# Alvin-Zeng/DRN

Measured on AMD Instinct MI355X. Metric: clips/sec fwd+bwd (BxT=256x4096 C3D feats), higher is better.
Workload: dtype bf16; 1 GPU; Charades-STA-shaped C3D features, T=256, D=4096, batch 32/GPU, stage-1 losses; step = fwd+bwd+grad all-reduce+clip(0.5)+Adam; global_batch=32, T=256, D=4096, parallelism=dp1

## Files before the change

drn_amd/csrc/api.hip:

```cpp
#include <stdarg.h>
#include "common.h"
#include "../../include/drn_hip.h"

static thread_local char g_err[512] = "";

void drn_set_error(const char* fmt, ...) {
  va_list ap;
  va_start(ap, fmt);
  vsnprintf(g_err, sizeof(g_err), fmt, ap);
  va_end(ap);
}

extern "C" int drn_abi_version(void) {
  drn_clear_status(); return DRN_ABI_VERSION; }
extern "C" const char* drn_last_error(void) { return g_err; }

static int g_tune[16] = {4096, 1, 256, 0, 0, 0, 0, 0, 1, 1, 0, 16, 160, 512, 2048, 1};
int drn_tuning(int key) { return g_tune[key]; }
extern "C" int drn_tune(const char* key, int value) {
  drn_clear_status();
  if (key && !strcmp(key, "tn3_minrows")) { g_tune[DRN_TUNE_TN3_MINROWS] = value; return DRN_OK; }
  if (key && !strcmp(key, "tn_fused")) { g_tune[DRN_TUNE_TN_FUSED] = value; return DRN_OK; }
  if (key && !strcmp(key, "nt_w4c")) { g_tune[DRN_TUNE_NT_W4C] = value; return DRN_OK; }
  if (key && !strcmp(key, "nt_w4")) { g_tune[DRN_TUNE_NT_W4] = value; return DRN_OK; }
  if (key && !strcmp(key, "nt_deep")) { g_tune[DRN_TUNE_NT_DEEP] = value; return DRN_OK; }
  if (key && !strcmp(key, "nt_w4h")) { g_tune[DRN_TUNE_NT_W4H] = value; return DRN_OK; }
  if (key && !strcmp(key, "w4h_tapil")) { g_tune[DRN_TUNE_W4H_TAPIL] = value; return DRN_OK; }
  if (key && !strcmp(key, "w4h_halo")) { g_tune[DRN_TUNE_W4H_HALO] = value; return DRN_OK; }
  if (key && !strcmp(key, "bn1_maxwg")) { g_tune[DRN_TUNE_BN1_MAXWG] = value; return DRN_OK; }
  if (key && !strcmp(key, "nt_deep2")) { g_tune[DRN_TUNE_NT_DEEP2] = value; return DRN_OK; }
  if (key && !strcmp(key, "nt_deep_ks")) { g_tune[DRN_TUNE_NT_DEEP_KS] = value; return DRN_OK; }
  if (key && !strncmp(key, "exp", 3) && key[3] >= '0' && key[3] <= '4' && !key[4]) { g_tune[DRN_TUNE_EXP0 + (key[3] - '0')] = value; return DRN_OK; }
  drn_set_error("drn_tune: unknown key %s", key ? key : "(null)");
  return DRN_ERR_ARG;
}
```

drn_amd/csrc/common.h:

```cpp
#pragma once
#include <hip/hip_runtime.h>
#include <stdint.h>
#include <stdio.h>
#include <string.h>

#define DRN_OK 0
#define DRN_ERR_ARG (-1)
#define DRN_ERR_LAUNCH (-2)
#define DRN_ERR_UNSUPPORTED (-3)

#define DRN_F32 0
#define DRN_BF16 1

typedef __bf16 bf16_t;
typedef __bf16 bf16x8 __attribute__((ext_vector_type(8)));
typedef __bf16 bf16x4 __attribute__((ext_vector_type(4)));
typedef short s16x4 __attribute__((ext_vector_type(4)));
typedef float f32x4 __attribute__((ext_vector_type(4)));
typedef float f32x2 __attribute__((ext_vector_type(2)));

template <typename T>
__device__ __forceinline__ T* as_global(T* p) {
  typedef __attribute__((address_space(1))) T* g_t;
  g_t g = (g_t)p;
  asm("" : "+s"(g));
  return (T*)g;
}
template <typename T>
__device__ __forceinline__ T* as_global_v(T* p) {
  typedef __attribute__((address_space(1))) T* g_t;
  g_t g = (g_t)p;
  asm("" : "+v"(g));
  return (T*)g;
}


void drn_set_error(const char* fmt, ...);

#define DRN_CHECK_ARG(cond, ...)          \
  do {                                    \
    if (!(cond)) {                        \
      drn_set_error(__VA_ARGS__);         \
      return DRN_ERR_ARG;                 \
    }                                     \
  } while (0)

static inline void drn_clear_status() { (void)hipGetLastError(); }

static inline int drn_launch_status(const char* what) {
  hipError_t e = hipGetLastError();
  if (e != hipSuccess) {
    drn_set_error("%s: launch failed: %s", what, hipGetErrorString(e));
    return DRN_ERR_LAUNCH;
  }
  return DRN_OK;
}

static inline int cdiv(int a, int b) { return (a + b - 1) / b; }

#ifdef DRN_EXPERIMENTS
#include <stdlib.h>
static inline const char* drn_exp_env(const char* name) { return getenv(name); }
#else
static inline const char* drn_exp_env(const char*) { return nullptr; }
#endif
int drn_tuning(int key);
#define DRN_XCHG_CONFIRM 0x20000
#define DRN_XCHG_READBACK 0x40000
#define DRN_XCHG_NONE 0x80000
#define DRN_TUNE_TN3_MINROWS 0
#define DRN_TUNE_TN_FUSED 1
#define DRN_TUNE_EXP0 3
#define DRN_TUNE_NT_W4C 9
#define DRN_TUNE_NT_W4 8
#define DRN_TUNE_NT_DEEP 2
#define DRN_TUNE_NT_W4H 12
#define DRN_TUNE_BN1_MAXWG 13
#define DRN_TUNE_W4H_TAPIL 14
#define DRN_TUNE_W4H_HALO 15
#define DRN_TUNE_NT_DEEP2 10
#define DRN_TUNE_NT_DEEP_KS 11

static __device__ uint4 g_zero_page[4];

template <typename T> struct DT;
template <> struct DT<float> {
  static __device__ __forceinline__ float ld(const float* p) { return *p; }
  static __device__ __forceinline__ void st(float* p, float v) { *p = v; }
  static __device__ __forceinline__ float round(float v) { return v; }
};
template <> struct DT<bf16_t> {
  static __device__ __forceinline__ float ld(const bf16_t* p) { return (float)*p; }
  static __device__ __forceinline__ void st(bf16_t* p, float v) { *p = (bf16_t)v; }
  static __device__ __forceinline__ float round(float v) { return (float)(bf16_t)v; }
};

__device__ __forceinline__ float wave_sum(float v) {
#pragma unroll
  for (int o = 32; o > 0; o >>= 1) v += __shfl_xor(v, o, 64);
  return v;
}

__device__ __forceinline__ float block_sum(float v, float* sh ) {
  v = wave_sum(v);
  const int w = threadIdx.x >> 6, l = threadIdx.x & 63, nw = blockDim.x >> 6;
  __syncthreads();
  if (l == 0) sh[w] = v;
  __syncthreads();
  if (w == 0) {
    float t = l < nw ? sh[l] : 0.f;
    t = wave_sum(t);
    if (l == 0) sh[16] = t;
  }
  __syncthreads();
  return sh[16];
}
```

drn_amd/csrc/gemm_tn.hip:

```cpp
#include <stdlib.h>
#include <type_traits>
#include "common.h"
#include "../../include/drn_hip.h"



struct WgradGroup {
  const void* dY;
  const void* X;
  int M, Lout, Lsrc, ldy, ldx;
  int blk_start;
};
struct WgradParams {
  int ngroups;
  WgradGroup g[DRN_MAX_GROUPS];
  int total_blks, blks_per_split;
  int N, Cin, taps, stride, pad;
  int ctiles;
  float* out;
  int direct;
  int w_layout;
  int accumulate;
  int multi;
  int z_start[DRN_MAX_GROUPS + 1], bps[DRN_MAX_GROUPS], gdirect[DRN_MAX_GROUPS];
// ... 238 lines not shown
        if (c >= Cin) continue;
        float v = acc[mi][ni][r];
        if (direct) {
          float* dst = P.w_layout == 0 ? out_ptr + ((long)n * KW + tap * Cin + c)
                                       : out_ptr + ((long)n * KW + (long)c * P.taps + tap);
          if (P.accumulate) v += *dst;
          *dst = v;
        } else {
          out_ptr[((long)split * P.N + n) * KW + tap * Cin + c] = v;
        }
      }
    }
}

__device__ __forceinline__ bf16x8 tr_frag(const char* lo_addr, const char* hi_addr) {
  typedef __attribute__((address_space(3))) s16x4* lp;
  union { struct { s16x4 a, b; } s; bf16x8 v; } u;
  u.s.a = __builtin_amdgcn_ds_read_tr16_b64_v4i16((lp)lo_addr);
  u.s.b = __builtin_amdgcn_ds_read_tr16_b64_v4i16((lp)hi_addr);
  return u.v;
}

template <int NSTG>
__global__ __launch_bounds__(512, 2) void conv_wgrad3_tn_kernel(const WgradParams P) {
  extern __shared__ __attribute__((aligned(16))) char smem[];
  typedef bf16_t T;
  constexpr int R = 64, MI = 4, NI = 2;
  constexpr int IMG = 16384, HALO_B = 512, STAGE_B = 2 * IMG + HALO_B;
  const int tid = threadIdx.x, w = __builtin_amdgcn_readfirstlane(tid >> 6), l = tid & 63;
  const int n0 = blockIdx.x * 128, c0 = blockIdx.y * 128;
  int split = blockIdx.z;
  int blk_lo = split * P.blks_per_split;
  int blk_hi = min(blk_lo + P.blks_per_split, P.total_blks);
  float* out_ptr = P.out;
  int direct = P.direct;
  if (P.multi) {
    int pg = 0;
#pragma unroll
    for (int i = 1; i < DRN_MAX_GROUPS; ++i)
      if (i < P.ngroups && (int)blockIdx.z >= P.z_start[i]) pg = i;
    split = blockIdx.z - P.z_start[pg];
    const int blk_end = pg + 1 < P.ngroups ? P.g[pg + 1].blk_start : P.total_blks;
    blk_lo = P.g[pg].blk_start + split * P.bps[pg];
    blk_hi = min(blk_lo + P.bps[pg], blk_end);
    out_ptr = P.gout[pg];
    direct = P.gdirect[pg];
  }
  const T* zero = (const T*)g_zero_page;

  const int srow = w * 8 + (l >> 3);
  const int scol = (((l & 7) >> 1) ^ ((srow >> 1) & 3)) * 16 + (l & 1) * 8;
  long y_off[2], x_off[2];
#pragma unroll
  for (int j = 0; j < 2; ++j) {
    y_off[j] = n0 + j * 64 + scol < P.N ? n0 + j * 64 + scol : -1;
    x_off[j] = c0 + j * 64 + scol < P.Cin ? c0 + j * 64 + scol : -1;
  }
  const bool is_halo = (w == 0) & (l < 32);
  const int hcol = ((l >> 3) & 1) * 64 + (l & 7) * 8;
  const long xh_off = c0 + hcol < P.Cin ? c0 + hcol : -1;
  const int rowoff[2] = {srow, (l >> 4) ? R : -1};
  int s_blk = blk_lo, s_g = 0;
#pragma unroll
  for (int i = 1; i < DRN_MAX_GROUPS; ++i)
    if (i < P.ngroups && blk_lo >= P.g[i].blk_start) s_g = i;
  int s_seq[2], s_t[2];
  const T* g_Y;
  const T* g_X;
  int g_L, g_nseq, g_ldy, g_ldx, g_next;
  auto locate = [&]() {
    const WgradGroup& G = P.g[s_g];
    g_Y = (const T*)G.dY;
    g_X = (const T*)G.X;
    g_L = G.Lout;
    g_nseq = G.M / G.Lout;
    g_ldy = G.ldy;
    g_ldx = G.ldx;
    g_next = s_g + 1 < P.ngroups ? P.g[s_g + 1].blk_start : 0x7fffffff;
    const int Lp = G.Lout + 1;
    const int pbase = (s_blk - G.blk_start) * R;
#pragma unroll
    for (int j = 0; j < 2; ++j) {
      const int p = pbase + rowoff[j] + Lp;
      const int q = p / Lp;
      s_seq[j] = q - 1;
      s_t[j] = p - q * Lp;
    }
  };
  locate();

  auto row_ptr = [&](const T* base, int m, int ld, long coff, bool ok) -> const T* {
    const unsigned off = __umul24((unsigned)m, (unsigned)ld) + (unsigned)coff;
    const T* p = base + off;
    return ok ? p : zero;
  };
  auto stage_part = [&](int buf, int part) {
    char* Ys = smem + buf * STAGE_B;
    char* Xs = Ys + IMG;
    char* Hs = Xs + IMG;
    const bool live = s_blk < blk_hi;
    const int L = g_L;
    const bool ok = live & ((unsigned)s_seq[0] < (unsigned)g_nseq) & (s_t[0] < L);
    const int m = s_seq[0] * L + s_t[0];
    if (part == 0) glds16(row_ptr(g_Y, m, g_ldy, y_off[0], ok & (y_off[0] >= 0)), Ys + w * 1024);
    if (part == 1) glds16(row_ptr(g_X, m, g_ldx, x_off[0], ok & (x_off[0] >= 0)), Xs + w * 1024);
    if (part == 2) glds16(row_ptr(g_Y, m, g_ldy, y_off[1], ok & (y_off[1] >= 0)), Ys + 8192 + w * 1024);
    if (part == 3) {
      glds16(row_ptr(g_X, m, g_ldx, x_off[1], ok & (x_off[1] >= 0)), Xs + 8192 + w * 1024);
      if (is_halo) {
        const bool okh = live & ((unsigned)s_seq[1] < (unsigned)g_nseq) & (s_t[1] < L) & (xh_off >= 0);
        glds16(row_ptr(g_X, s_seq[1] * L + s_t[1], g_ldx, xh_off, okh), Hs);
      }
    }
    if (part != 4) return;
    ++s_blk;
    if (s_blk >= g_next) {
      ++s_g;
      locate();
    } else {
      const int Lp = L + 1;
      if (Lp > R) {
#pragma unroll
        for (int j = 0; j < 2; ++j) {
          s_t[j] += R;
          const bool wrap = s_t[j] >= Lp;
          s_t[j] -= wrap ? Lp : 0;
          s_seq[j] += wrap ? 1 : 0;
        }
      } else {
#pragma unroll
        for (int j = 0; j < 2; ++j) {
          s_t[j] += R;
          while (s_t[j] >= Lp) {
            s_t[j] -= Lp;
            ++s_seq[j];
          }
        }
      }
    }
  };
  auto stage = [&](int buf) {
#pragma unroll
    for (int part = 0; part < 5; ++part) stage_part(buf, part);
  };

  f32x4 acc[3][MI][NI];
#pragma unroll
  for (int t = 0; t < 3; ++t)
#pragma unroll
    for (int mi = 0; mi < MI; ++mi)
#pragma unroll
      for (int ni = 0; ni < NI; ++ni) acc[t][mi][ni] = (f32x4){0.f, 0.f, 0.f, 0.f};
  const int wr = w >> 2, wc = w & 3;

  const int fr = (l >> 4) * 4 + ((l & 15) >> 2);
  const int fb = (l & 3) * 8;
  int ya[MI], xa[3][NI], x_first[NI], x_last[NI];
#pragma unroll
  for (int mi = 0; mi < MI; ++mi) ya[mi] = wr * 8192 + fr * 128 + ((mi ^ ((fr >> 1) & 3)) * 32) + fb;
#pragma unroll
  for (int ni = 0; ni < NI; ++ni) {
    const int half = wc >> 1, cb = (wc & 1) * 2 + ni;
#pragma unroll
    for (int t = 0; t < 3; ++t) {
      const int rr = fr + t - 1;
      xa[t][ni] = IMG + half * 8192 + rr * 128 + ((cb ^ ((rr >> 1) & 3)) * 32) + fb;
    }
    x_first[ni] = fr == 0 ? 2 * IMG + half * 128 + cb * 32 + fb : xa[0][ni];
    x_last[ni] = fr == 15 ? 2 * IMG + 256 + half * 128 + cb * 32 + fb : xa[2][ni] + 4096 + 2048;
  }

  struct Frags {
    bf16x8 a[MI], b[3][NI];
  };
  auto load_frags = [&](Frags& F, const char* S, auto ks_) {
    constexpr int ks = decltype(ks_)::value;
#pragma unroll
    for (int mi = 0; mi < MI; ++mi) {
      const char* q = S + ya[mi] + ks * 4096;
      F.a[mi] = tr_frag(q, q + 2048);
    }
#pragma unroll
    for (int ni = 0; ni < NI; ++ni) {
      const char* q0 = S + xa[0][ni] + ks * 4096;
      const char* q1 = S + xa[1][ni] + ks * 4096;
      const char* q2 = S + xa[2][ni] + ks * 4096;
      F.b[1][ni] = tr_frag(q1, q1 + 2048);
      F.b[0][ni] = tr_frag(ks == 0 ? S + x_first[ni] : q0, q0 + 2048);
      F.b[2][ni] = tr_frag(q2, ks == 1 ? S + x_last[ni] : q2 + 2048);
    }
  };
  auto mfma_frags = [&](const Frags& F, int mi0) {
#pragma unroll
    for (int t = 0; t < 3; ++t)
#pragma unroll
      for (int mi = 0; mi < 2; ++mi)
#pragma unroll
        for (int ni = 0; ni < NI; ++ni)
          acc[t][mi0 + mi][ni] = __builtin_amdgcn_mfma_f32_16x16x32_bf16(F.a[mi0 + mi], F.b[t][ni], acc[t][mi0 + mi][ni], 0, 0, 0);
  };
  typedef std::integral_constant<int, 0> K0;
  typedef std::integral_constant<int, 1> K1;

  auto wait_landed = [&](int younger) {
    if (younger <= 0) asm volatile("s_waitcnt vmcnt(0)" ::: "memory");
    else if (younger == 1) { if (w == 0) asm volatile("s_waitcnt vmcnt(5)" ::: "memory"); else asm volatile("s_waitcnt vmcnt(4)" ::: "memory"); }
    else { if (w == 0) asm volatile("s_waitcnt vmcnt(10)" ::: "memory"); else asm volatile("s_waitcnt vmcnt(8)" ::: "memory"); }
  };
#pragma unroll
  for (int st = 0; st < NSTG - 1; ++st) stage(st);
  wait_landed(NSTG - 2);
  __builtin_amdgcn_s_barrier();
  asm volatile("" ::: "memory");
  Frags F0, F1;
  load_frags(F0, smem, K0());
  int cur = 0;
  for (int blk = blk_lo; blk < blk_hi; ++blk) {
    wait_landed(NSTG - 3);
    __builtin_amdgcn_s_barrier();
    asm volatile("" ::: "memory");
    int nxt = cur + NSTG - 1;
    if (nxt >= NSTG) nxt -= NSTG;
    const int cn = cur + 1 == NSTG ? 0 : cur + 1;
    load_frags(F1, smem + cur * STAGE_B, K1());
    stage_part(nxt, 0);
    __builtin_amdgcn_sched_barrier(0);
    mfma_frags(F0, 0);
    __builtin_amdgcn_sched_barrier(0);
    stage_part(nxt, 1);
    __builtin_amdgcn_sched_barrier(0);
    mfma_frags(F0, 2);
    __builtin_amdgcn_sched_barrier(0);
    load_frags(F0, smem + cn * STAGE_B, K0());
    stage_part(nxt, 2);
    __builtin_amdgcn_sched_barrier(0);
    mfma_frags(F1, 0);
    __builtin_amdgcn_sched_barrier(0);
    stage_part(nxt, 3);
    __builtin_amdgcn_sched_barrier(0);
    mfma_frags(F1, 2);
    __builtin_amdgcn_sched_barrier(0);
    stage_part(nxt, 4);
    cur = cn;
  }
  asm volatile("s_waitcnt vmcnt(0)" ::: "memory");

  const int KW = 3 * P.Cin;
  const bool rowmajor = !direct || (P.w_layout == 0 && !P.accumulate);
  float* obase = direct ? out_ptr : out_ptr + (long)split * P.N * KW;
  if (rowmajor && (P.Cin % 4 == 0) && (((uintptr_t)obase & 15) == 0)) {
    constexpr int PITCH = 32 * 4 + 16;
    __syncthreads();
    char* wbuf = smem + w * (32 * PITCH);
#pragma unroll
    for (int t = 0; t < 3; ++t)
#pragma unroll
      for (int ch = 0; ch < MI / 2; ++ch) {
        const int nrow0 = n0 + wr * 64 + ch * 32;
#pragma unroll
        for (int mi2 = 0; mi2 < 2; ++mi2)
#pragma unroll
          for (int r = 0; r < 4; ++r)
#pragma unroll
            for (int ni = 0; ni < NI; ++ni)
              *((float*)(wbuf + (mi2 * 16 + (l >> 4) * 4 + r) * PITCH) + ni * 16 + (l & 15)) = acc[t][ch * 2 + mi2][ni][r];
        asm volatile("s_waitcnt lgkmcnt(0)" ::: "memory");
#pragma unroll
        for (int it = 0; it < 4; ++it) {
          const int rl = it * 8 + (l >> 3), cv = l & 7;
          const int n = nrow0 + rl, c = c0 + wc * 32 + cv * 4;
          if (n < P.N && c < P.Cin) {
            const f32x4 v = *(const f32x4*)(wbuf + rl * PITCH + cv * 16);
            *(f32x4*)(obase + ((long)n * KW + t * P.Cin + c)) = v;
          }
        }
        asm volatile("s_waitcnt lgkmcnt(0)" ::: "memory");
      }
    return;
  }
#pragma unroll
  for (int t = 0; t < 3; ++t)
#pragma unroll
    for (int mi = 0; mi < MI; ++mi)
#pragma unroll
      for (int r = 0; r < 4; ++r) {
        const int n = n0 + wr * 64 + mi * 16 + (l >> 4) * 4 + r;
        if (n >= P.N) continue;
#pragma unroll
        for (int ni = 0; ni < NI; ++ni) {
          const int c = c0 + wc * 32 + ni * 16 + (l & 15);
          if (c >= P.Cin) continue;
          float v = acc[t][mi][ni][r];
          if (direct) {
            float* dst = P.w_layout == 0 ? out_ptr + ((long)n * KW + t * P.Cin + c) : out_ptr + ((long)n * KW + (long)c * 3 + t);
            if (P.accumulate) v += *dst;
            *dst = v;
          } else {
            out_ptr[((long)split * P.N + n) * KW + t * P.Cin + c] = v;
          }
        }
      }
}

struct WgradReduceMulti {
  const float* ws[DRN_MAX_GROUPS];
  float* out[DRN_MAX_GROUPS];
  int nsplit[DRN_MAX_GROUPS];
  int cin[DRN_MAX_GROUPS];
};
__global__ void wgrad_reduce_multi_kernel(const WgradReduceMulti R, int N, int taps, int w_layout, int accumulate) {
  const int Cin = R.cin[blockIdx.y];
  const long KW = (long)taps * Cin;
  const long total = (long)N * KW;
  const float* __restrict__ ws = R.ws[blockIdx.y];
  float* __restrict__ out = R.out[blockIdx.y];
  const int nsplit = R.nsplit[blockIdx.y];
  if (nsplit <= 1) return;
  if (w_layout == 1 && taps == 3) {
    const long pairs = (long)N * Cin;
    for (long idx = (long)blockIdx.x * blockDim.x + threadIdx.x; idx < pairs; idx += (long)gridDim.x * blockDim.x) {
      const long n = idx / Cin;
      const int c = (int)(idx - n * Cin);
      const float* p = ws + n * KW + c;
      float s0 = 0.f, s1 = 0.f, s2 = 0.f;
#pragma unroll 4
      for (int z = 0; z < nsplit; ++z) {
        s0 += p[(long)z * total];
        s1 += p[(long)z * total + Cin];
        s2 += p[(long)z * total + 2 * Cin];
      }
      float* o = out + n * KW + (long)c * 3;
      if (accumulate) {
        s0 += o[0];
        s1 += o[1];
        s2 += o[2];
      }
      o[0] = s0;
      o[1] = s1;
      o[2] = s2;
    }
    return;
  }
  for (long idx = (long)blockIdx.x * blockDim.x + threadIdx.x; idx < total; idx += (long)gridDim.x * blockDim.x) {
    float s = 0.f;
    for (int z = 0; z < nsplit; ++z) s += ws[(long)z * total + idx];
    long o = idx;
    if (w_layout == 1) {
      const long n = idx / KW;
      const int rem = (int)(idx - n * KW);
      const int tap = rem / Cin, c = rem - tap * Cin;
      o = n * KW + (long)c * taps + tap;
    }
    if (accumulate) s += out[o];
    out[o] = s;
  }
}

__global__ void wgrad_reduce_kernel(const float* __restrict__ ws, float* __restrict__ out, int nsplit, int N, int Cin,
                                    int taps, int w_layout, int accumulate) {
  const long KW = (long)taps * Cin;
  const long total = (long)N * KW;
  if (w_layout == 1 && taps == 3) {
    const long pairs = (long)N * Cin;
    for (long idx = (long)blockIdx.x * blockDim.x + threadIdx.x; idx < pairs; idx += (long)gridDim.x * blockDim.x) {
      const long n = idx / Cin;
      const int c = (int)(idx - n * Cin);
      const float* p = ws + n * KW + c;
      float s0 = 0.f, s1 = 0.f, s2 = 0.f;
#pragma unroll 4
      for (int z = 0; z < nsplit; ++z) {
        s0 += p[(long)z * total];
        s1 += p[(long)z * total + Cin];
        s2 += p[(long)z * total + 2 * Cin];
      }
      float* o = out + n * KW + (long)c * 3;
      if (accumulate) {
        s0 += o[0];
        s1 += o[1];
        s2 += o[2];
      }
      o[0] = s0;
      o[1] = s1;
      o[2] = s2;
    }
    return;
  }
  for (long idx = (long)blockIdx.x * blockDim.x + threadIdx.x; idx < total; idx += (long)gridDim.x * blockDim.x) {
    float s = 0.f;
    for (int z = 0; z < nsplit; ++z) s += ws[(long)z * total + idx];
    long o = idx;
    if (w_layout == 1) {
      const long n = idx / KW;
      const int rem = (int)(idx - n * KW);
      const int tap = rem / Cin, c = rem - tap * Cin;
      o = n * KW + (long)c * taps + tap;
    }
    if (accumulate) s += out[o];
    out[o] = s;
  }
}

typedef DrnWgradPendItem WgradPendItem;
#define WGRAD_PEND_MAX DRN_WGRAD_PEND_MAX
typedef DrnWgradPending WgradPendParams;

static int wgrad_pend_push(DrnWgradPending* L, const float* ws, float* out, int nsplit, int N, int Cin, int taps, int w_layout, int accumulate) {
  if (!L || L->n < 0 || L->n >= WGRAD_PEND_MAX) return 0;
  for (int i = 0; i < L->n; ++i)
    if (L->it[i].out == out) {
      drn_set_error("drn_gemm_wgrad: the output already has a deferred reduce pending in this DrnWgradPending (flush with drn_wgrad_reduce_pending first)");
      return DRN_ERR_ARG;
    }
  if (accumulate) return 0;
  L->it[L->n++] = WgradPendItem{ws, out, nsplit, N, Cin, taps, w_layout, accumulate};
  return 1;
}

__global__ __launch_bounds__(256) void wgrad_reduce_all_kernel(const WgradPendParams P) {
  __shared__ float sh_sq[17];
  float sq = 0.f;
  int i = 0;
  for (int k = 1; k < P.n; ++k)
    if ((int)blockIdx.x >= P.blk_start[k]) i = k;
  const WgradPendItem& I = P.it[i];
  const int nb = P.blk_start[i + 1] - P.blk_start[i], b = blockIdx.x - P.blk_start[i];
  const float* __restrict__ ws = I.ws;
  float* __restrict__ out = I.out;
  const int N = I.N, Cin = I.Cin, taps = I.taps, nsplit = I.nsplit, accumulate = I.accumulate, w_layout = I.w_layout;
  const long KW = (long)taps * Cin;
  const long total = (long)N * KW;
  if (w_layout == 1 && taps == 3) {
    const long pairs = (long)N * Cin;
    for (long idx = (long)b * 256 + threadIdx.x; idx < pairs; idx += (long)nb * 256) {
      const long n = idx / Cin;
      const int c = (int)(idx - n * Cin);
      const float* p = ws + n * KW + c;
      float s0 = 0.f, s1 = 0.f, s2 = 0.f;
#pragma unroll 4
      for (int z = 0; z < nsplit; ++z) {
        s0 += __builtin_nontemporal_load(p + (long)z * total);
        s1 += __builtin_nontemporal_load(p + (long)z * total + Cin);
        s2 += __builtin_nontemporal_load(p + (long)z * total + 2 * Cin);
      }
      float* o = out + n * KW + (long)c * 3;
      if (accumulate) {
        s0 += o[0];
        s1 += o[1];
        s2 += o[2];
      }
      o[0] = s0;
      o[1] = s1;
      o[2] = s2;
      sq = fmaf(s0, s0, sq); sq = fmaf(s1, s1, sq); sq = fmaf(s2, s2, sq);
    }
  } else {
    for (long idx = (long)b * 256 + threadIdx.x; idx < total; idx += (long)nb * 256) {
      float s = 0.f;
      for (int z = 0; z < nsplit; ++z) s += __builtin_nontemporal_load(ws + (long)z * total + idx);
      long o = idx;
      if (w_layout == 1) {
        const long n = idx / KW;
        const int rem = (int)(idx - n * KW);
        const int tap = rem / Cin, c = rem - tap * Cin;
        o = n * KW + (long)c * taps + tap;
      }
      if (accumulate) s += out[o];
      out[o] = s;
      sq = fmaf(s, s, sq);
    }
  }
  if (P.sumsq) {
    sq = block_sum(sq, sh_sq);
    if (threadIdx.x == 0) P.sumsq[blockIdx.x] = sq;
  }
}

static int wgrad_pend_plan(DrnWgradPending* L) {
  int blocks = 0;
  for (int i = 0; i < L->n; ++i) {
    const WgradPendItem& I = L->it[i];
    const long work = (I.w_layout == 1 && I.taps == 3) ? (long)I.N * I.Cin : (long)I.N * I.taps * I.Cin;
    int nb = (int)((work + 255) / 256);
    if (nb > 2048) nb = 2048;
    L->blk_start[i] = blocks;
    blocks += nb;
  }
  L->blk_start[L->n] = blocks;
  return blocks;
}

extern "C" int drn_wgrad_pending_blocks(DrnWgradPending* L) {
  drn_clear_status();
  DRN_CHECK_ARG(L && L->n >= 0 && L->n <= WGRAD_PEND_MAX, "drn_wgrad_pending_blocks: bad list");
  return wgrad_pend_plan(L);
}

extern "C" int64_t drn_wgrad_pending_bytes(const DrnWgradPending* L) {
  int64_t b = 0;
  if (!L || L->n < 0 || L->n > WGRAD_PEND_MAX) return 0;
  for (int i = 0; i < L->n; ++i) {
    const WgradPendItem& I = L->it[i];
    b += (int64_t)I.N * I.taps * I.Cin * 4 * (I.nsplit + 1 + (I.accumulate ? 1 : 0));
  }
  return b;
}

extern "C" int drn_wgrad_reduce_pending(DrnWgradPending* L, float* sumsq, void* stream) {
  drn_clear_status();
  DRN_CHECK_ARG(L && L->n >= 0 && L->n <= WGRAD_PEND_MAX, "drn_wgrad_reduce_pending: bad list");
  if (L->n == 0) return DRN_OK;
  const int blocks = wgrad_pend_plan(L);
  L->sumsq = sumsq;
  wgrad_reduce_all_kernel<<<blocks, 256, 0, (hipStream_t)stream>>>(*L);
  L->n = 0;
  L->sumsq = nullptr;
  return drn_launch_status("drn_wgrad_reduce_pending");
}

static int wgrad_tile(int N, int Cin, int taps) {
  if (const char* e = drn_exp_env("DRN_TN_TILE")) return atoi(e) == 256 ? 256 : 128;
  return (long)cdiv(N, 256) * taps * cdiv(Cin, 256) >= 128 ? 256 : 128;
}

static int wgrad_nsplit(int total_blks, int N, int Cin, int taps) {
  const int tile = wgrad_tile(N, Cin, taps);
  const int tiles = cdiv(N, tile) * taps * cdiv(Cin, tile);
  const int tgt = drn_tuning(DRN_TUNE_EXP0 + 2) > 0 ? drn_tuning(DRN_TUNE_EXP0 + 2) : 768;
  int ns = cdiv(tile == 256 ? 256 : tgt, tiles);
  const int cap = total_blks / 12;
  if (ns > cap) ns = cap;
  if (ns < 1) ns = 1;
  if (ns > 64) ns = 64;
  return ns;
}

static int total_blocks_upper(int M_total, int ngroups_max) {
  return cdiv(M_total, 32) + ngroups_max;
}

static int wgrad3_nsplit(int m_total, int N, int Cin) {
  int target = drn_tuning(DRN_TUNE_EXP0 + 1) > 0 ? drn_tuning(DRN_TUNE_EXP0 + 1) : 256;
  if (const char* e = drn_exp_env("DRN_TN3_TARGET")) target = atoi(e);
  const int tiles = cdiv(N, 128) * cdiv(Cin, 128);
  int ns = target / tiles;
  const int cap = cdiv(m_total, 64) / 8;
  if (ns > cap) ns = cap;
  if (ns < 1) ns = 1;
  if (ns > 64) ns = 64;
  return ns;
}
static bool wgrad3_enabled() {
  return drn_tuning(DRN_TUNE_TN_FUSED) != 0;
}
static bool wgrad3_group_ok(const DrnWgradDesc& s) {
  return s.Lsrc == s.Lout && s.M < (1 << 24) && s.ldy < (1 << 24) && s.ldx < (1 << 24) &&
         (long)s.M * s.ldy < (1L << 31) && (long)s.M * s.ldx < (1L << 31);
}
static int wgrad3_min_rows() {
  return drn_tuning(DRN_TUNE_TN3_MINROWS);
}
static void wgrad3_attr() {
  static bool set = false;
  if (!set) {
#ifdef DRN_EXPERIMENTS
    (void)hipFuncSetAttribute((const void*)conv_wgrad3_tn_kernel<3>, hipFuncAttributeMaxDynamicSharedMemorySize, 163840);
#endif
    (void)hipFuncSetAttribute((const void*)conv_wgrad3_tn_kernel<4>, hipFuncAttributeMaxDynamicSharedMemorySize, 163840);
    set = true;
  }
}
#define WGRAD3_STAGE (2 * 16384 + 512)
static int wgrad3_stages() {
  int st = 4;
  if (const char* e = drn_exp_env("DRN_TN3_STAGES")) st = atoi(e);
  return st < 3 ? 3 : (st > 4 ? 4 : st);
}
#ifdef DRN_EXPERIMENTS
#define WGRAD3_LAUNCH(GRID, P) do { const int st_ = wgrad3_stages(); \
    if (st_ == 3) conv_wgrad3_tn_kernel<3><<<GRID, 512, 3 * WGRAD3_STAGE, stream>>>(P); \
    else conv_wgrad3_tn_kernel<4><<<GRID, 512, 4 * WGRAD3_STAGE, stream>>>(P); } while (0)
#else
#define WGRAD3_LAUNCH(GRID, P) conv_wgrad3_tn_kernel<4><<<GRID, 512, 4 * WGRAD3_STAGE, stream>>>(P)
#endif

extern "C" int64_t drn_wgrad_ws_elems(int M_total, int N, int Cin, int taps) {
  int ns = wgrad_nsplit(total_blocks_upper(M_total, DRN_MAX_GROUPS), N, Cin, taps);
  if (taps == 3) {
    const int ns3 = wgrad3_nsplit(M_total, N, Cin);
    if (ns3 > ns) ns = ns3;
  }
  return ns > 1 ? (int64_t)ns * N * taps * Cin : 0;
}

extern "C" int drn_gemm_wgrad(const DrnWgradDesc* d, int ngroups, float* dW, int N, int Cin, int taps, int stride, int pad,
                              int w_layout, int accumulate, float* ws, int dtype, DrnWgradPending* pend, void* stream_) {
  drn_clear_status();
  hipStream_t stream = (hipStream_t)stream_;
  DRN_CHECK_ARG(ngroups >= 1 && ngroups <= DRN_MAX_GROUPS, "drn_gemm_wgrad: ngroups=%d out of range", ngroups);
  DRN_CHECK_ARG(dtype == DRN_F32 || dtype == DRN_BF16, "drn_gemm_wgrad: bad dtype %d", dtype);
  DRN_CHECK_ARG(dW && N > 0 && Cin > 0 && taps >= 1 && stride >= 1, "drn_gemm_wgrad: bad dims");
  if (pend)
    for (int i = 0; i < pend->n && i < WGRAD_PEND_MAX; ++i)
      DRN_CHECK_ARG(pend->it[i].out != dW, "drn_gemm_wgrad: the output already has a deferred reduce pending in this DrnWgradPending (flush first)");
  const int ch = dtype == DRN_BF16 ? 8 : 4;
  const int R = dtype == DRN_BF16 ? 64 : 32;
  WgradParams P;
  memset(&P, 0, sizeof(P));
  P.ngroups = ngroups;
  int blks = 0, m_total = 0;
  for (int g = 0; g < ngroups; ++g) {
    const DrnWgradDesc& s = d[g];
    DRN_CHECK_ARG(s.dY && s.X && s.M > 0 && s.Lout > 0 && s.Lsrc > 0 && s.M % s.Lout == 0, "drn_gemm_wgrad: bad group %d", g);
    DRN_CHECK_ARG(s.ldy % ch == 0 && s.ldx % ch == 0 && N % ch == 0 && Cin % ch == 0,
                  "drn_gemm_wgrad: N/Cin/ldy/ldx must be multiples of %d elements", ch);
    DRN_CHECK_ARG(((uintptr_t)s.dY & 15) == 0 && ((uintptr_t)s.X & 15) == 0, "drn_gemm_wgrad: operands must be 16-byte aligned");
    P.g[g].dY = s.dY; P.g[g].X = s.X; P.g[g].M = s.M; P.g[g].Lout = s.Lout; P.g[g].Lsrc = s.Lsrc;
    P.g[g].ldy = s.ldy; P.g[g].ldx = s.ldx; P.g[g].blk_start = blks;
    blks += cdiv(s.M, R);
    m_total += s.M;
  }
  bool fused = dtype == DRN_BF16 && taps == 3 && stride == 1 && pad == 1 && wgrad3_enabled() && m_total >= wgrad3_min_rows();
  for (int g = 0; g < ngroups; ++g) fused = fused && wgrad3_group_ok(d[g]);
  if (fused) {
    blks = 0;
    for (int g = 0; g < ngroups; ++g) {
      P.g[g].blk_start = blks;
      blks += cdiv((d[g].M / d[g].Lout) * (d[g].Lout + 1), 64);
    }
    int ns = wgrad3_nsplit(m_total, N, Cin);
    if (ns > blks) ns = blks;
    DRN_CHECK_ARG(ns == 1 || ws, "drn_gemm_wgrad: workspace required (drn_wgrad_ws_elems)");
    P.total_blks = blks;
    P.blks_per_split = cdiv(blks, ns);
    ns = cdiv(blks, P.blks_per_split);
    P.N = N; P.Cin = Cin; P.taps = taps; P.stride = stride; P.pad = pad;
    P.ctiles = cdiv(Cin, 128);
    P.direct = ns == 1;
    P.out = P.direct ? dW : ws;
    P.w_layout = w_layout;
    P.accumulate = accumulate;
    wgrad3_attr();
    WGRAD3_LAUNCH(dim3(cdiv(N, 128), cdiv(Cin, 128), ns), P);
    int rc = drn_launch_status("drn_gemm_wgrad(fused taps)");
    if (rc) return rc;
    const int pushed = P.direct ? 0 : wgrad_pend_push(pend, ws, dW, ns, N, Cin, taps, w_layout, accumulate);
    if (pushed < 0) return pushed;
    if (!P.direct && !pushed) {
      const long total = (long)N * taps * Cin;
      int nb = (int)((total + 255) / 256);
      if (nb > 2048) nb = 2048;
      wgrad_reduce_kernel<<<nb, 256, 0, stream>>>(ws, dW, ns, N, Cin, taps, w_layout, accumulate);
      rc = drn_launch_status("drn_gemm_wgrad(reduce)");
    }
    return rc;
  }
  int ns = wgrad_nsplit(total_blocks_upper(m_total, DRN_MAX_GROUPS), N, Cin, taps);
  if (ns > blks) ns = blks;
  DRN_CHECK_ARG(ns == 1 || ws, "drn_gemm_wgrad: workspace required (drn_wgrad_ws_elems)");
  P.total_blks = blks;
  P.blks_per_split = cdiv(blks, ns);
  ns = cdiv(blks, P.blks_per_split);
  P.N = N; P.Cin = Cin; P.taps = taps; P.stride = stride; P.pad = pad;
  const int tile = wgrad_tile(N, Cin, taps);
  P.ctiles = cdiv(Cin, tile);
  P.direct = ns == 1;
  P.out = P.direct ? dW : ws;
  P.w_layout = w_layout;
  P.accumulate = accumulate;
  static bool attr_set = false;
  if (!attr_set) {
    (void)hipFuncSetAttribute((const void*)conv_wgrad_tn_kernel<float, 2, 2, 4, 4>, hipFuncAttributeMaxDynamicSharedMemorySize, 163840);
    (void)hipFuncSetAttribute((const void*)conv_wgrad_tn_kernel<bf16_t, 2, 2, 4, 4>, hipFuncAttributeMaxDynamicSharedMemorySize, 163840);
    (void)hipFuncSetAttribute((const void*)conv_wgrad_tn_kernel<float, 2, 4, 8, 4>, hipFuncAttributeMaxDynamicSharedMemorySize, 163840);
    (void)hipFuncSetAttribute((const void*)conv_wgrad_tn_kernel<bf16_t, 2, 4, 8, 4>, hipFuncAttributeMaxDynamicSharedMemorySize, 163840);
    (void)hipFuncSetAttribute((const void*)conv_wgrad_tn_kernel<float, 2, 4, 4, 2>, hipFuncAttributeMaxDynamicSharedMemorySize, 163840);
    (void)hipFuncSetAttribute((const void*)conv_wgrad_tn_kernel<bf16_t, 2, 4, 4, 2>, hipFuncAttributeMaxDynamicSharedMemorySize, 163840);
    attr_set = true;
  }
  dim3 grid(cdiv(N, tile), taps * P.ctiles, ns);
  if (tile == 256) {
    if (dtype == DRN_BF16) conv_wgrad_tn_kernel<bf16_t, 2, 4, 8, 4><<<grid, 512, 2 * 65536, stream>>>(P);
    else conv_wgrad_tn_kernel<float, 2, 4, 8, 4><<<grid, 512, 2 * 65536, stream>>>(P);
  } else {
#ifdef DRN_EXPERIMENTS
    if (drn_exp_env("DRN_TN_WAVES") && atoi(drn_exp_env("DRN_TN_WAVES")) == 4) {
      if (dtype == DRN_BF16) conv_wgrad_tn_kernel<bf16_t, 2, 2, 4, 4><<<grid, 256, 2 * 32768, stream>>>(P);
      else conv_wgrad_tn_kernel<float, 2, 2, 4, 4><<<grid, 256, 2 * 32768, stream>>>(P);
    } else
#endif
    if (dtype == DRN_BF16) conv_wgrad_tn_kernel<bf16_t, 2, 4, 4, 2><<<grid, 512, 2 * 32768, stream>>>(P);
    else conv_wgrad_tn_kernel<float, 2, 4, 4, 2><<<grid, 512, 2 * 32768, stream>>>(P);
  }
  int rc = drn_launch_status("drn_gemm_wgrad");
  if (rc) return rc;
  const int pushed = P.direct ? 0 : wgrad_pend_push(pend, ws, dW, ns, N, Cin, taps, w_layout, accumulate);
  if (pushed < 0) return pushed;
  if (!P.direct && !pushed) {
    const long total = (long)N * taps * Cin;
    int nb = (int)((total + 255) / 256);
    if (nb > 2048) nb = 2048;
    wgrad_reduce_kernel<<<nb, 256, 0, stream>>>(ws, dW, ns, N, Cin, taps, w_layout, accumulate);
    rc = drn_launch_status("drn_gemm_wgrad(reduce)");
  }
  return rc;
}

extern "C" int drn_gemm_wgrad_multi(const DrnWgradDesc* d, int n, float* const* dWs, int N, int Cin, const int32_t* Cins, int taps,
                                    int stride, int pad, int w_layout, int accumulate, float* ws, int dtype, DrnWgradPending* pend,
                                    void* stream_) {
  drn_clear_status();
  hipStream_t stream = (hipStream_t)stream_;
  DRN_CHECK_ARG(d && dWs && n >= 1 && n <= DRN_MAX_GROUPS, "drn_gemm_wgrad_multi: n=%d out of range", n);
  if (pend)
    for (int g = 0; g < n; ++g)
      for (int i = 0; i < pend->n && i < WGRAD_PEND_MAX; ++i)
        DRN_CHECK_ARG(pend->it[i].out != dWs[g], "drn_gemm_wgrad_multi: output %d already has a deferred reduce pending in this DrnWgradPending", g);
  DRN_CHECK_ARG(dtype == DRN_F32 || dtype == DRN_BF16, "drn_gemm_wgrad_multi: bad dtype %d", dtype);
  DRN_CHECK_ARG(N > 0 && Cin > 0 && taps >= 1 && stride >= 1, "drn_gemm_wgrad_multi: bad dims");
  const int ch = dtype == DRN_BF16 ? 8 : 4;
  const int R = dtype == DRN_BF16 ? 64 : 32;
  const int tile = 128;
  WgradParams P;
  WgradReduceMulti RM;
  memset(&P, 0, sizeof(P));
  memset(&RM, 0, sizeof(RM));
  P.ngroups = n;
  P.multi = 1;
  bool varied = false;
  for (int g = 0; g < n && Cins; ++g) {
    DRN_CHECK_ARG(Cins[g] > 0 && Cins[g] <= Cin && Cins[g] % ch == 0, "drn_gemm_wgrad_multi: bad Cins[%d]", g);
    varied |= Cins[g] != Cin;
  }
  int blks = 0, z = 0, mmax = 0;
  bool any_split = false;
  for (int g = 0; g < n; ++g) mmax = d[g].M > mmax ? d[g].M : mmax;
  const long ws_per = drn_wgrad_ws_elems(mmax, N, Cin, taps);
  bool fused = !varied && dtype == DRN_BF16 && taps == 3 && stride == 1 && pad == 1 && wgrad3_enabled() && mmax >= wgrad3_min_rows();
  for (int g = 0; g < n; ++g) fused = fused && wgrad3_group_ok(d[g]);
  for (int g = 0; g < n; ++g) {
    const DrnWgradDesc& s = d[g];
    DRN_CHECK_ARG(s.dY && s.X && dWs[g] && s.M > 0 && s.Lout > 0 && s.Lsrc > 0 && s.M % s.Lout == 0, "drn_gemm_wgrad_multi: bad problem %d", g);
    DRN_CHECK_ARG(s.ldy % ch == 0 && s.ldx % ch == 0 && N % ch == 0 && Cin % ch == 0,
                  "drn_gemm_wgrad_multi: N/Cin/ldy/ldx must be multiples of %d elements", ch);
    DRN_CHECK_ARG(((uintptr_t)s.dY & 15) == 0 && ((uintptr_t)s.X & 15) == 0, "drn_gemm_wgrad_multi: operands must be 16-byte aligned");
    P.g[g].dY = s.dY; P.g[g].X = s.X; P.g[g].M = s.M; P.g[g].Lout = s.Lout; P.g[g].Lsrc = s.Lsrc;
    P.g[g].ldy = s.ldy; P.g[g].ldx = s.ldx; P.g[g].blk_start = blks;
    const int gb = fused ? cdiv((s.M / s.Lout) * (s.Lout + 1), 64) : cdiv(s.M, R);
    blks += gb;
    const int cin_g = Cins ? Cins[g] : Cin;
    const long per = (long)N * taps * cin_g;
    P.gcin[g] = cin_g; RM.cin[g] = cin_g;
    int ns = wgrad_nsplit(total_blocks_upper(s.M, 1), N, cin_g, taps);
    if (fused) {
      long m_all = 0;
      for (int k = 0; k < n; ++k) m_all += d[k].M;
      ns = (int)((long)wgrad3_nsplit(mmax, N, Cin) * s.M / m_all);
      const int cap = gb / 4;
      if (ns > cap) ns = cap;
      if (ns < 1) ns = 1;
    }
    if (ns > gb) ns = gb;
    P.bps[g] = cdiv(gb, ns);
    ns = cdiv(gb, P.bps[g]);
    DRN_CHECK_ARG(ns == 1 || ws, "drn_gemm_wgrad_multi: workspace required");
    P.z_start[g] = z;
    z += ns;
    P.gdirect[g] = ns == 1;
    P.gout[g] = ns == 1 ? dWs[g] : ws + (long)g * ws_per;
    RM.ws[g] = ws + (long)g * ws_per; RM.out[g] = dWs[g]; RM.nsplit[g] = ns;
    any_split |= ns > 1;
    DRN_CHECK_ARG(ns == 1 || (long)ns * per <= ws_per, "drn_gemm_wgrad_multi: workspace slice too small");
  }
  P.z_start[n] = z;
  P.total_blks = blks;
  P.blks_per_split = blks;
  P.N = N; P.Cin = Cin; P.taps = taps; P.stride = stride; P.pad = pad;
  P.ctiles = cdiv(Cin, tile);
  P.w_layout = w_layout;
  P.accumulate = accumulate;
  static bool attr_set = false;
  if (!attr_set) {
    (void)hipFuncSetAttribute((const void*)conv_wgrad_tn_kernel<float, 2, 4, 4, 2>, hipFuncAttributeMaxDynamicSharedMemorySize, 163840);
    (void)hipFuncSetAttribute((const void*)conv_wgrad_tn_kernel<bf16_t, 2, 4, 4, 2>, hipFuncAttributeMaxDynamicSharedMemorySize, 163840);
    attr_set = true;
  }
  dim3 grid(cdiv(N, tile), taps * P.ctiles, z);
  if (fused) {
    wgrad3_attr();
    WGRAD3_LAUNCH(dim3(cdiv(N, 128), cdiv(Cin, 128), z), P);
  } else if (dtype == DRN_BF16) conv_wgrad_tn_kernel<bf16_t, 2, 4, 4, 2><<<grid, 512, 2 * 32768, stream>>>(P);
  else conv_wgrad_tn_kernel<float, 2, 4, 4, 2><<<grid, 512, 2 * 32768, stream>>>(P);
  int rc = drn_launch_status("drn_gemm_wgrad_multi");
  if (rc || !any_split) return rc;
  if (pend && !accumulate && pend->n >= 0 && pend->n + n <= WGRAD_PEND_MAX) {
    for (int g = 0; g < n; ++g)
      if (RM.nsplit[g] > 1) (void)wgrad_pend_push(pend, RM.ws[g], RM.out[g], RM.nsplit[g], N, RM.cin[g], taps, w_layout, accumulate);
    return rc;
  }
  int nb = (int)(((long)N * taps * Cin + 255) / 256);
  if (nb > 1024) nb = 1024;
  wgrad_reduce_multi_kernel<<<dim3(nb, n), 256, 0, stream>>>(RM, N, taps, w_layout, accumulate);
  return drn_launch_status("drn_gemm_wgrad_multi(reduce)");
}
```

Before: 17580 clips/s.

## Add warp-specialized wgrad3 kernel with dedicated producer waves for async loads

```diff
diff --git a/drn_amd/csrc/api.hip b/drn_amd/csrc/api.hip
--- a/drn_amd/csrc/api.hip
+++ b/drn_amd/csrc/api.hip
@@ -20,7 +20,8 @@
 extern "C" int drn_tune(const char* key, int value) {
   drn_clear_status();
   if (key && !strcmp(key, "tn3_minrows")) { g_tune[DRN_TUNE_TN3_MINROWS] = value; return DRN_OK; }
-  if (key && !strcmp(key, "tn_fused")) { g_tune[DRN_TUNE_TN_FUSED] = value; return DRN_OK; }
+  if (key && !strcmp(key, "tn_fused")) { g_tune[DRN_TUNE_TN_FUSED] = (g_tune[DRN_TUNE_TN_FUSED] & DRN_TN3_SCHED_OLD) | (value & ~DRN_TN3_SCHED_OLD); return DRN_OK; }
+  if (key && !strcmp(key, "tn3_sched")) { g_tune[DRN_TUNE_TN_FUSED] = (g_tune[DRN_TUNE_TN_FUSED] & ~DRN_TN3_SCHED_OLD) | (value ? 0 : DRN_TN3_SCHED_OLD); return DRN_OK; }
   if (key && !strcmp(key, "nt_w4c")) { g_tune[DRN_TUNE_NT_W4C] = value; return DRN_OK; }
   if (key && !strcmp(key, "nt_w4")) { g_tune[DRN_TUNE_NT_W4] = value; return DRN_OK; }
   if (key && !strcmp(key, "nt_deep")) { g_tune[DRN_TUNE_NT_DEEP] = value; return DRN_OK; }
diff --git a/drn_amd/csrc/common.h b/drn_amd/csrc/common.h
--- a/drn_amd/csrc/common.h
+++ b/drn_amd/csrc/common.h
@@ -70,6 +70,7 @@
 #define DRN_XCHG_NONE 0x80000
 #define DRN_TUNE_TN3_MINROWS 0
 #define DRN_TUNE_TN_FUSED 1
+#define DRN_TN3_SCHED_OLD 0x100
 #define DRN_TUNE_EXP0 3
 #define DRN_TUNE_NT_W4C 9
 #define DRN_TUNE_NT_W4 8
diff --git a/drn_amd/csrc/gemm_tn.hip b/drn_amd/csrc/gemm_tn.hip
--- a/drn_amd/csrc/gemm_tn.hip
+++ b/drn_amd/csrc/gemm_tn.hip
@@ -564,6 +564,273 @@
       }
 }
 
+__global__ __launch_bounds__(768, 1) void conv_wgrad3_ws_kernel(const WgradParams P) {
+  extern __shared__ __attribute__((aligned(16))) char smem[];
+  typedef bf16_t T;
+  constexpr int R = 64, MI = 4, NI = 2, NSTG = 4;
+  constexpr int IMG = 16384, HALO_B = 512, STAGE_B = 2 * IMG + HALO_B;
+  const int tid = threadIdx.x, w = __builtin_amdgcn_readfirstlane(tid >> 6), l = tid & 63;
+  const int n0 = blockIdx.x * 128, c0 = blockIdx.y * 128;
+  int split = blockIdx.z;
+  int blk_lo = split * P.blks_per_split;
+  int blk_hi = min(blk_lo + P.blks_per_split, P.total_blks);
+  float* out_ptr = P.out;
+  int direct = P.direct;
+  if (P.multi) {
+    int pg = 0;
+#pragma unroll
+    for (int i = 1; i < DRN_MAX_GROUPS; ++i)
+      if (i < P.ngroups && (int)blockIdx.z >= P.z_start[i]) pg = i;
+    split = blockIdx.z - P.z_start[pg];
+    const int blk_end = pg + 1 < P.ngroups ? P.g[pg + 1].blk_start : P.total_blks;
+    blk_lo = P.g[pg].blk_start + split * P.bps[pg];
+    blk_hi = min(blk_lo + P.bps[pg], blk_end);
+    out_ptr = P.gout[pg];
+    direct = P.gdirect[pg];
+  }
+
+  if (w >= 8) {
+    const T* zero = (const T*)g_zero_page;
+    const int p = w - 8;
+    int rowoff[3];
+    long y_off[2][2], x_off[2][2];
+#pragma unroll
+    for (int k = 0; k < 2; ++k) {
+      const int srow = (2 * p + k) * 8 + (l >> 3);
+      const int scol = (((l & 7) >> 1) ^ ((srow >> 1) & 3)) * 16 + (l & 1) * 8;
+      rowoff[k] = srow;
+#pragma unroll
+      for (int j = 0; j < 2; ++j) {
+        y_off[k][j] = n0 + j * 64 + scol < P.N ? n0 + j * 64 + scol : -1;
+        x_off[k][j] = c0 + j * 64 + scol < P.Cin ? c0 + j * 64 + scol : -1;
+      }
+    }
+    rowoff[2] = (l >> 4) ? R : -1;
+    const bool is_halo = (p == 0) & (l < 32);
+    const int hcol = ((l >> 3) & 1) * 64 + (l & 7) * 8;
+    const long xh_off = c0 + hcol < P.Cin ? c0 + hcol : -1;
+    int s_blk = blk_lo, s_g = 0;
+#pragma unroll
+    for (int i = 1; i < DRN_MAX_GROUPS; ++i)
+      if (i < P.ngroups && blk_lo >= P.g[i].blk_start) s_g = i;
+    int s_seq[3], s_t[3];
+    const T* g_Y;
+    const T* g_X;
+    int g_L, g_nseq, g_ldy, g_ldx, g_next;
+    auto locate = [&]() {
+      const WgradGroup& G = P.g[s_g];
+      g_Y = (const T*)G.dY;
+      g_X = (const T*)G.X;
+      g_L = G.Lout;
+      g_nseq = G.M / G.Lout;
+      g_ldy = G.ldy;
+      g_ldx = G.ldx;
+      g_next = s_g + 1 < P.ngroups ? P.g[s_g + 1].blk_start : 0x7fffffff;
+      const int Lp = G.Lout + 1;
+      const int pbase = (s_blk - G.blk_start) * R;
+#pragma unroll
+      for (int j = 0; j < 3; ++j) {
+        const int pp = pbase + rowoff[j] + Lp;
+        const int q = pp / Lp;
+        s_seq[j] = q - 1;
+        s_t[j] = pp - q * Lp;
+      }
+    };
+    locate();
+    auto row_ptr = [&](const T* base, int m, int ld, long coff, bool ok) -> const T* {
+      const unsigned off = __umul24((unsigned)m, (unsigned)ld) + (unsigned)coff;
+      const T* ptr = base + off;
+      return ok ? ptr : zero;
+    };
+    auto stage = [&](int buf) {
+      char* Ys = smem + buf * STAGE_B;
+      char* Xs = Ys + IMG;
+      char* Hs = Xs + IMG;
+      const bool live = s_blk < blk_hi;
+      const int L = g_L;
+#pragma unroll
+      for (int k = 0; k < 2; ++k) {
+        const bool ok = live & ((unsigned)s_seq[k] < (unsigned)g_nseq) & (s_t[k] < L);
+        const int m = s_seq[k] * L + s_t[k];
+        const int piece = (2 * p + k) * 1024;
+        glds16(row_ptr(g_Y, m, g_ldy, y_off[k][0], ok & (y_off[k][0] >= 0)), Ys + piece);
+        glds16(row_ptr(g_X, m, g_ldx, x_off[k][0], ok & (x_off[k][0] >= 0)), Xs + piece);
+        glds16(row_ptr(g_Y, m, g_ldy, y_off[k][1], ok & (y_off[k][1] >= 0)), Ys + 8192 + piece);
+        glds16(row_ptr(g_X, m, g_ldx, x_off[k][1], ok & (x_off[k][1] >= 0)), Xs + 8192 + piece);
+      }
+      if (is_halo) {
+        const bool okh = live & ((unsigned)s_seq[2] < (unsigned)g_nseq) & (s_t[2] < L) & (xh_off >= 0);
+        glds16(row_ptr(g_X, s_seq[2] * L + s_t[2], g_ldx, xh_off, okh), Hs);
+      }
+      ++s_blk;
+      if (s_blk >= g_next) {
+        ++s_g;
+        locate();
+      } else {
+        const int Lp = L + 1;
+        if (Lp > R) {
+#pragma unroll
+          for (int j = 0; j < 3; ++j) {
+            s_t[j] += R;
+            const bool wrap = s_t[j] >= Lp;
+            s_t[j] -= wrap ? Lp : 0;
+            s_seq[j] += wrap ? 1 : 0;
+          }
+        } else {
+#pragma unroll
+          for (int j = 0; j < 3; ++j) {
+            s_t[j] += R;
+            while (s_t[j] >= Lp) {
+              s_t[j] -= Lp;
+              ++s_seq[j];
+            }
+          }
+        }
+      }
+    };
+#pragma unroll
+    for (int st = 0; st < NSTG - 1; ++st) stage(st);
+    int nxt = NSTG - 1;
+    for (int blk = blk_lo; blk < blk_hi; ++blk) {
+      if (p == 0) asm volatile("s_waitcnt vmcnt(18)" ::: "memory");
+      else asm volatile("s_waitcnt vmcnt(16)" ::: "memory");
+      __builtin_amdgcn_s_barrier();
+      asm volatile("" ::: "memory");
+      stage(nxt);
+      nxt = nxt + 1 == NSTG ? 0 : nxt + 1;
+    }
+    asm volatile("s_waitcnt vmcnt(0)" ::: "memory");
+    __syncthreads();
+    return;
+  }
+
+  const int wr = w >> 2, wc = w & 3;
+  const int fr = (l >> 4) * 4 + ((l & 15) >> 2);
+  const int fb = (l & 3) * 8;
+  int ya[MI], xa[3][NI], x_first[NI], x_last[NI];
+#pragma unroll
+  for (int mi = 0; mi < MI; ++mi) ya[mi] = wr * 8192 + fr * 128 + ((mi ^ ((fr >> 1) & 3)) * 32) + fb;
+#pragma unroll
+  for (int ni = 0; ni < NI; ++ni) {
+    const int half = wc >> 1, cb = (wc & 1) * 2 + ni;
+#pragma unroll
+    for (int t = 0; t < 3; ++t) {
+      const int rr = fr + t - 1;
+      xa[t][ni] = IMG + half * 8192 + rr * 128 + ((cb ^ ((rr >> 1) & 3)) * 32) + fb;
+    }
+    x_first[ni] = fr == 0 ? 2 * IMG + half * 128 + cb * 32 + fb : xa[0][ni];
+    x_last[ni] = fr == 15 ? 2 * IMG + 256 + half * 128 + cb * 32 + fb : xa[2][ni] + 4096 + 2048;
+  }
+  f32x4 acc[3][MI][NI];
+#pragma unroll
+  for (int t = 0; t < 3; ++t)
+#pragma unroll
+    for (int mi = 0; mi < MI; ++mi)
+#pragma unroll
+      for (int ni = 0; ni < NI; ++ni) acc[t][mi][ni] = (f32x4){0.f, 0.f, 0.f, 0.f};
+  struct Frags {
+    bf16x8 a[MI], b[3][NI];
+  };
+  auto load_frags = [&](Frags& F, const char* S, auto ks_) {
+    constexpr int ks = decltype(ks_)::value;
+#pragma unroll
+    for (int mi = 0; mi < MI; ++mi) {
+      const char* q = S + ya[mi] + ks * 4096;
+      F.a[mi] = tr_frag(q, q + 2048);
+    }
+#pragma unroll
+    for (int ni = 0; ni < NI; ++ni) {
+      const char* q0 = S + xa[0][ni] + ks * 4096;
+      const char* q1 = S + xa[1][ni] + ks * 4096;
+      const char* q2 = S + xa[2][ni] + ks * 4096;
+      F.b[1][ni] = tr_frag(q1, q1 + 2048);
+      F.b[0][ni] = tr_frag(ks == 0 ? S + x_first[ni] : q0, q0 + 2048);
+      F.b[2][ni] = tr_frag(q2, ks == 1 ? S + x_last[ni] : q2 + 2048);
+    }
+  };
+  auto mfma_frags = [&](const Frags& F) {
+#pragma unroll
+    for (int mi0 = 0; mi0 < MI; mi0 += 2)
+#pragma unroll
+      for (int t = 0; t < 3; ++t)
+#pragma unroll
+        for (int mi = 0; mi < 2; ++mi)
+#pragma unroll
+          for (int ni = 0; ni < NI; ++ni)
+            acc[t][mi0 + mi][ni] = __builtin_amdgcn_mfma_f32_16x16x32_bf16(F.a[mi0 + mi], F.b[t][ni], acc[t][mi0 + mi][ni], 0, 0, 0);
+  };
+  typedef std::integral_constant<int, 0> K0;
+  typedef std::integral_constant<int, 1> K1;
+  int cur = 0;
+  for (int blk = blk_lo; blk < blk_hi; ++blk) {
+    __builtin_amdgcn_s_barrier();
+    asm volatile("" ::: "memory");
+    const char* S = smem + cur * STAGE_B;
+    Frags F;
+    load_frags(F, S, K0());
+    mfma_frags(F);
+    load_frags(F, S, K1());
+    mfma_frags(F);
+    cur = cur + 1 == NSTG ? 0 : cur + 1;
+  }
+  __syncthreads();
+
+  const int KW = 3 * P.Cin;
+  const bool rowmajor = !direct || (P.w_layout == 0 && !P.accumulate);
+  float* obase = direct ? out_ptr : out_ptr + (long)split * P.N * KW;
+  if (rowmajor && (P.Cin % 4 == 0) && (((uintptr_t)obase & 15) == 0)) {
+    constexpr int PITCH = 32 * 4 + 16;
+    char* wbuf = smem + w * (32 * PITCH);
+#pragma unroll
+    for (int t = 0; t < 3; ++t)
+#pragma unroll
+      for (int ch = 0; ch < MI / 2; ++ch) {
+        const int nrow0 = n0 + wr * 64 + ch * 32;
+#pragma unroll
+        for (int mi2 = 0; mi2 < 2; ++mi2)
+#pragma unroll
+          for (int r = 0; r < 4; ++r)
+#pragma unroll
+            for (int ni = 0; ni < NI; ++ni)
+              *((float*)(wbuf + (mi2 * 16 + (l >> 4) * 4 + r) * PITCH) + ni * 16 + (l & 15)) = acc[t][ch * 2 + mi2][ni][r];
+        asm volatile("s_waitcnt lgkmcnt(0)" ::: "memory");
+#pragma unroll
+        for (int it = 0; it < 4; ++it) {
+          const int rl = it * 8 + (l >> 3), cv = l & 7;
+          const int n = nrow0 + rl, c = c0 + wc * 32 + cv * 4;
+          if (n < P.N && c < P.Cin) {
+            const f32x4 v = *(const f32x4*)(wbuf + rl * PITCH + cv * 16);
+            *(f32x4*)(obase + ((long)n * KW + t * P.Cin + c)) = v;
+          }
+        }
+        asm volatile("s_waitcnt lgkmcnt(0)" ::: "memory");
+      }
+    return;
+  }
+#pragma unroll
+  for (int t = 0; t < 3; ++t)
+#pragma unroll
+    for (int mi = 0; mi < MI; ++mi)
+#pragma unroll
+      for (int r = 0; r < 4; ++r) {
+        const int n = n0 + wr * 64 + mi * 16 + (l >> 4) * 4 + r;
+        if (n >= P.N) continue;
+#pragma unroll
+        for (int ni = 0; ni < NI; ++ni) {
+          const int c = c0 + wc * 32 + ni * 16 + (l & 15);
+          if (c >= P.Cin) continue;
+          float v = acc[t][mi][ni][r];
+          if (direct) {
+            float* dst = P.w_layout == 0 ? out_ptr + ((long)n * KW + t * P.Cin + c) : out_ptr + ((long)n * KW + (long)c * 3 + t);
+            if (P.accumulate) v += *dst;
+            *dst = v;
+          } else {
+            out_ptr[((long)split * P.N + n) * KW + t * P.Cin + c] = v;
+          }
+        }
+      }
+}
+
 struct WgradReduceMulti {
   const float* ws[DRN_MAX_GROUPS];
   float* out[DRN_MAX_GROUPS];
@@ -812,7 +1079,7 @@
   return ns;
 }
 static bool wgrad3_enabled() {
-  return drn_tuning(DRN_TUNE_TN_FUSED) != 0;
+  return (drn_tuning(DRN_TUNE_TN_FUSED) & ~DRN_TN3_SCHED_OLD) != 0;
 }
 static bool wgrad3_group_ok(const DrnWgradDesc& s) {
   return s.Lsrc == s.Lout && s.M < (1 << 24) && s.ldy < (1 << 24) && s.ldx < (1 << 24) &&
@@ -828,6 +1095,7 @@
     (void)hipFuncSetAttribute((const void*)conv_wgrad3_tn_kernel<3>, hipFuncAttributeMaxDynamicSharedMemorySize, 163840);
 #endif
     (void)hipFuncSetAttribute((const void*)conv_wgrad3_tn_kernel<4>, hipFuncAttributeMaxDynamicSharedMemorySize, 163840);
+    (void)hipFuncSetAttribute((const void*)conv_wgrad3_ws_kernel, hipFuncAttributeMaxDynamicSharedMemorySize, 163840);
     set = true;
   }
 }
@@ -838,12 +1106,15 @@
   return st < 3 ? 3 : (st > 4 ? 4 : st);
 }
 #ifdef DRN_EXPERIMENTS
-#define WGRAD3_LAUNCH(GRID, P) do { const int st_ = wgrad3_stages(); \
+#define WGRAD3_LAUNCH_OLD(GRID, P) do { const int st_ = wgrad3_stages(); \
     if (st_ == 3) conv_wgrad3_tn_kernel<3><<<GRID, 512, 3 * WGRAD3_STAGE, stream>>>(P); \
     else conv_wgrad3_tn_kernel<4><<<GRID, 512, 4 * WGRAD3_STAGE, stream>>>(P); } while (0)
 #else
-#define WGRAD3_LAUNCH(GRID, P) conv_wgrad3_tn_kernel<4><<<GRID, 512, 4 * WGRAD3_STAGE, stream>>>(P)
+#define WGRAD3_LAUNCH_OLD(GRID, P) conv_wgrad3_tn_kernel<4><<<GRID, 512, 4 * WGRAD3_STAGE, stream>>>(P)
 #endif
+#define WGRAD3_LAUNCH(GRID, P) do { \
+    if (drn_tuning(DRN_TUNE_TN_FUSED) & DRN_TN3_SCHED_OLD) WGRAD3_LAUNCH_OLD(GRID, P); \
+    else conv_wgrad3_ws_kernel<<<GRID, 768, 4 * WGRAD3_STAGE, stream>>>(P); } while (0)
 
 extern "C" int64_t drn_wgrad_ws_elems(int M_total, int N, int Cin, int taps) {
   int ns = wgrad_nsplit(total_blocks_upper(M_total, DRN_MAX_GROUPS), N, Cin, taps);
```

After: 17670 clips/s (median of 6 runs). Within noise of the previous version (+0.5%).
